# ofsouzap/DistributedMandelbrot

Hardware: AMD Instinct MI355X
Metric: G pixel-iterations/s on 4096^2 tile, max_iter=1000 fp64 (higher is better)
Workload: dtype f64

## Files before the change

### distributedmandelbrot_amd/_lib.py

```python
from __future__ import annotations

import ctypes as C
import importlib.util
import os
import sys

HERE = os.path.dirname(os.path.abspath(__file__))
SO_PATH = os.path.join(HERE, "libmbk_hip.so")

MBK_OK, MBK_ERR_INVALID, MBK_ERR_NO_DEVICE, MBK_ERR_HIP, MBK_ERR_NOMEM, MBK_ERR_NET = range(6)
MBK_WANT_COUNTS = 0x1
MBK_WANT_BYTES = 0x2
MBK_KERNEL_DEFAULT = 0x000
MBK_KERNEL_SIMPLE = 0x100
MBK_KERNEL_ASM = 0x200
MBK_KERNEL_REFILL = 0x300
MBK_KERNEL_GROUP = 0x400
MBK_KERNEL_SCAN = 0x500
KERNELS = {"default": MBK_KERNEL_DEFAULT, "simple": MBK_KERNEL_SIMPLE, "asm": MBK_KERNEL_ASM,
           "refill": MBK_KERNEL_REFILL, "group": MBK_KERNEL_GROUP, "scan": MBK_KERNEL_SCAN}
OPTIONS = {name: i for i, name in enumerate(
    ["order", "waves_per_wg", "group_steps", "exact_steps", "probe_steps", "scan_waves", "scan_xcd_map", "scan_col_period", "heavy_share",
     "rf_livemin", "rf_patience", "rf_batch", "rf_waves", "cycle_detect", "probe_mid", "prepass_overlap", "exact_long", "scan_inline", "wave_limit", "units_min_light", "xcd_balance", "m_late", "h_settled", "classify_wg", "scan_strip", "cycle_window", "spill_first", "spill_lanes", "spill_min_mrd", "spill_min_blocks", "spill_cyc_shift",
     "sure_interior"])}
MBK_PRECISION_F32 = 0x1000
MBK_LAZY_UNIFORM = 0x2000
MBK_DEEP_BLA = 0x8000
MBK_DEEP_XBLA = 0x10000
PRECISIONS = {"f64": 0, "f32": MBK_PRECISION_F32}
MBK_SLOTS = 4
MBK_WORKER_DEPTH = 3
MBK_INFO_SCAN_WG_PER_CU = 100
MBK_INFO_XCD_SHARE = 110
MBK_INFO_SPILL = 130
MBK_CODEC_RAW = 0x00
MBK_CODEC_RLE = 0x01
MBK_CHUNK_DEFINITION = 4096
MBK_CHUNK_BYTES = 4096 * 4096
MBK_ABI_VERSION = 5
MBK_RENDER_BYTES = 0
MBK_RENDER_SMOOTH = 1
MBK_RENDER_DISTANCE = 3
MBK_RENDER_DISTANCE_REL = 4
MBK_RENDER_EQUALIZED = 5
RENDER_SOURCES = {"bytes": MBK_RENDER_BYTES, "smooth": MBK_RENDER_SMOOTH, "distance": MBK_RENDER_DISTANCE,
                  "distance_rel": MBK_RENDER_DISTANCE_REL, "equalized": MBK_RENDER_EQUALIZED}
MBK_HISTOGRAM_MAX_MRD = 1 << 20
# ... 131 lines not shown
    "mbk_view_launch_distance": (C.c_int, [C.c_void_p, C.POINTER(mbk_view), C.c_uint32, C.c_uint32,
                                           C.c_void_p, C.c_void_p, C.c_void_p]),
    "mbk_view_compute_distance": (C.c_int, [C.c_void_p, C.POINTER(mbk_view), C.c_uint32, C.c_uint32,
                                            C.c_void_p, C.c_void_p, C.POINTER(mbk_stats)]),
    "mbk_distance_value_host": (C.c_double, [C.c_double, C.c_double, C.c_int32]),
    "mbk_datachunk_submit": (C.c_int, [C.c_void_p, C.c_int, C.c_uint32, C.c_uint32, C.c_uint32, C.c_uint32,
                                       C.c_void_p, C.c_void_p]),
    "mbk_datachunk_submit_ex": (C.c_int, [C.c_void_p, C.c_int, C.c_uint32, C.c_uint32, C.c_uint32, C.c_uint32,
                                          C.c_void_p, C.c_void_p, C.c_uint32]),
    "mbk_view_submit": (C.c_int, [C.c_void_p, C.c_int, C.POINTER(mbk_view), C.c_uint32, C.c_uint32,
                                  C.c_void_p, C.c_void_p]),
    "mbk_wait": (C.c_int, [C.c_void_p, C.c_int, C.POINTER(mbk_stats)]),
    "mbk_serialize_last": (C.c_int, [C.c_void_p, C.c_void_p, C.c_uint64, C.POINTER(C.c_uint64),
                                     C.POINTER(C.c_uint32)]),
    "mbk_set_option": (C.c_int, [C.c_void_p, C.c_int, C.c_uint32]),
    "mbk_get_option": (C.c_int, [C.c_void_p, C.c_int, C.POINTER(C.c_uint32)]),
    "mbk_quantise_counts": (C.c_int, [C.c_void_p, C.c_void_p, C.c_uint64, C.c_uint32, C.c_void_p]),
    "mbk_units_plan": (C.c_int, [C.c_uint32, C.c_uint32, C.c_uint32, C.c_void_p, C.c_void_p]),
    "mbk_units_lookup": (C.c_int, [C.c_void_p, C.c_uint32, C.c_void_p, C.c_void_p]),
    "mbk_sure_interior_point": (C.c_int, [C.c_double, C.c_double]),
    "mbk_sure_interior_blocks": (C.c_int, [C.POINTER(mbk_view), C.POINTER(C.c_uint64)]),
    "mbk_sure_interior_flag": (C.c_int, [C.POINTER(mbk_view), C.c_uint32, C.c_uint32, C.c_uint32, C.c_uint32,
                                         C.POINTER(C.c_uint32)]),
    "mbk_reduce_counts": (C.c_int, [C.c_void_p, C.c_void_p, C.c_uint64, C.c_uint32, C.c_void_p,
                                    C.POINTER(mbk_stats)]),
    "mbk_worker_run": (C.c_int, [C.c_void_p, C.c_char_p, C.c_uint16, C.c_uint64, C.c_uint32,
                                 C.POINTER(mbk_worker_report)]),
    "mbk_net_set_option": (C.c_int, [C.c_int, C.c_uint32]),
    "mbk_net_get_option": (C.c_int, [C.c_int, C.POINTER(C.c_uint32)]),
    "mbk_feeder_run": (C.c_int, [C.POINTER(mbk_feeder_ops), C.c_char_p, C.c_uint16, C.c_uint64, C.c_uint32,
                                 C.POINTER(mbk_worker_report)]),
    "mbk_deep_orbit_create": (C.c_int, [C.c_char_p, C.c_char_p, C.c_uint32, C.c_uint32, C.POINTER(C.c_void_p)]),
    "mbk_deep_orbit_destroy": (None, [C.c_void_p]),
    "mbk_deep_orbit_info": (C.c_int, [C.c_void_p, C.POINTER(C.c_uint32), C.POINTER(C.c_uint32), C.POINTER(C.c_uint32),
                                      C.POINTER(C.c_uint32)]),
    "mbk_deep_orbit_read": (C.c_int, [C.c_void_p, C.c_void_p, C.c_void_p, C.c_uint64]),
    "mbk_deep_view_launch": (C.c_int, [C.c_void_p, C.c_void_p, C.POINTER(mbk_deep_view), C.c_uint32, C.c_uint32,
                                       C.c_void_p, C.c_void_p, C.c_void_p, C.c_void_p]),
    "mbk_deep_view_compute": (C.c_int, [C.c_void_p, C.c_void_p, C.POINTER(mbk_deep_view), C.c_uint32, C.c_uint32,
                                        C.c_void_p, C.c_void_p, C.c_void_p, C.POINTER(mbk_stats)]),
    "mbk_deep_view_submit": (C.c_int, [C.c_void_p, C.c_int, C.c_void_p, C.POINTER(mbk_deep_view), C.c_uint32, C.c_uint32,
                                       C.c_void_p, C.c_void_p]),
    "mbk_deep_view_launch_distance": (C.c_int, [C.c_void_p, C.c_void_p, C.POINTER(mbk_deep_view), C.c_uint32, C.c_uint32,
                                                C.c_void_p, C.c_void_p, C.c_void_p]),
    "mbk_deep_view_compute_distance": (C.c_int, [C.c_void_p, C.c_void_p, C.POINTER(mbk_deep_view), C.c_uint32, C.c_uint32,
                                                 C.c_void_p, C.c_void_p, C.POINTER(mbk_stats)]),
# ... 299 lines not shown
```

### distributedmandelbrot_amd/csrc/mbk_api.hip

```cpp
#include "../../include/mbk.h"

#include <hip/hip_runtime.h>

#include <cmath>
#include <cstdio>
#include <cstdlib>
#include <algorithm>
#include <cstring>
#include <new>
#include <string>
#include <vector>

#include "mbk_kernels.h"
#include "mbk_refill.h"
#include "mbk_persist.h"
#include "mbk_scan.h"
#include "mbk_units.h"
#include "mbk_spill.h"
#include "mbk_feeder.h"
#include "mbk_deep_orbit.h"
#include "mbk_deep.h"
#include "mbk_deep_bla.h"
#include "mbk_deep_wide.h"
#include "mbk_deep_wide_bla.h"
#include "mbk_histogram.h"
// ... 4 lines not shown
#include "mbk_interior.h"
#include "mbk_deep_distance.h"
#include "mbk_deep_distance_bla.h"
#include "mbk_deep_relief.h"
#include "mbk_deep_nucleus.h"
#include "mbk_deep_wide_nucleus.h"
#include "mbk_deep_wide_distance_bla.h"
#include "mbk_deep_wide_relief.h"
#include "mbk_deep_wide_distance.h"
#include "mbk_julia.h"
#include "mbk_julia_distance.h"
#include "mbk_density.h"
#include "mbk_adaptive.h"
#include "mbk_deep_adaptive.h"
#include "mbk_deep_wide_adaptive.h"

using mbk::Axis;
using mbk::ReduceOut;
using mbk::ReduceSlot;
using mbk::TileArgs;
using mbk::WorkQueues;
using mbk::kSafeImagMin;

static const int kOrderRing = 3;

struct OrderRing {
    uint32_t *d_order[kOrderRing] = {};
    uint32_t *d_capture = nullptr;
    uint32_t *d_ctl = nullptr;
    bool ctl_dirty = true;
    size_t order_cap = 0;
    unsigned order_turn = 0;
    hipStream_t aux = nullptr;
    uint32_t aux_prio = 0;
    int pp_last = -1;
    hipEvent_t ev_cls[kOrderRing] = {};
    hipEvent_t ev_done[kOrderRing] = {};
    bool done_valid[kOrderRing] = {};

    void drop_lists()
    {
        for (int k = 0; k < kOrderRing; ++k) {
            if (d_order[k]) (void)hipFree(d_order[k]);
            d_order[k] = nullptr;
            done_valid[k] = false;
        }
        if (d_capture) (void)hipFree(d_capture);
        d_capture = nullptr;
        order_cap = 0;
    }
    void drop_aux()
    {
        if (aux) (void)hipStreamDestroy(aux);
        aux = nullptr;
        for (int k = 0; k < kOrderRing; ++k) {
            if (ev_cls[k]) (void)hipEventDestroy(ev_cls[k]);
            if (ev_done[k]) (void)hipEventDestroy(ev_done[k]);
            ev_cls[k] = ev_done[k] = nullptr;
            done_valid[k] = false;
        }
    }
    void release()
    {
        if (aux) (void)hipStreamSynchronize(aux);
        drop_lists();
        drop_aux();
        if (d_ctl) (void)hipFree(d_ctl);
        *this = OrderRing();
    }
};

struct SpillBuffers {
    void *d_z = nullptr;
    uint32_t *d_meta = nullptr, *d_cnt = nullptr, *d_chunks = nullptr, *d_src = nullptr;
    unsigned long long *d_total = nullptr;
    size_t cap_slots = 0, cap_blocks = 0;

    void release()
    {
        for (void *q : {d_z, (void *)d_meta, (void *)d_cnt, (void *)d_chunks, (void *)d_src, (void *)d_total})
            if (q) (void)hipFree(q);
        *this = SpillBuffers();
    }
// ... 428 lines not shown
    p.order_mode = ctx->opt[MBK_OPT_ORDER];
    p.probe_steps = ctx->opt[MBK_OPT_PROBE_STEPS];
    a.perm_mul = p.order_mode == 1 ? coprime_multiplier(p.grid.x) : 1u;
    a.order = nullptr;
    p.units = p.order_mode == 3 && p.wpw == 1u && kernel == MBK_KERNEL_GROUP && !safe && a.smooth == nullptr &&
              (a.counts || a.bytes) && !(a.bytes && a.quant_wide) && a.blocks_x % 8u == 0u && a.blocks_x <= 2048u &&
              a.fast_bx_end > 0u && a.fast_by_end > 0u && (f32 || ctx->opt[MBK_OPT_GROUP_STEPS] == 16u) &&
              p.grid.x >= 16384u && (uint32_t)a.mrd > 2u * p.probe_steps && p.by <= 0xffffu;
    p.unit_share = 0.0;
    if (p.units) {
        p.unit_share = window_heavy_share(ctx, a);
        p.units = (1.0 - p.unit_share) * 65536.0 >= (double)ctx->opt[MBK_OPT_UNITS_MIN_LIGHT];
    }
    p.ordered = p.order_mode >= 2 && p.grid.x >= 16384u && (uint32_t)a.mrd > 2u * p.probe_steps && a.blocks_x <= 0xffffu && p.by <= 0xffffu;
    return p;
}

struct OrderList {
    StreamScratch *sc = nullptr;
    unsigned k = 0;
    uint32_t *list = nullptr;
    hipStream_t pre = nullptr;
    bool overlap = false;
    bool whole = false;
    ~OrderList() { if (sc && !whole) sc->ring.ctl_dirty = true; }
};

static const char *capture_list_missing(const OrderRing &ring, uint32_t nblocks, bool units)
{
    if (nblocks > ring.order_cap || !ring.d_capture)
        return "the stream's dispatch lists must grow for this window: make the same call, or a larger one, once outside the capture";
    if (units && (!ring.d_ctl || ring.ctl_dirty))
        return "the units pre-pass' counters must be cleared behind a drain: make the same call once outside the capture";
    return nullptr;
}

static bool capture_list_ready(const mbk_ctx *ctx, hipStream_t stream, uint32_t nblocks, bool units)
{
    for (const StreamScratch &sc : ctx->scratch)
        if (sc.stream == stream) return capture_list_missing(sc.ring, nblocks, units) == nullptr;
    return false;
}

static int acquire_order_list(mbk_ctx *ctx, hipStream_t stream, uint32_t nblocks, bool units, OrderList *out)
{
    StreamScratch *sc = nullptr;
    int rc = get_scratch(ctx, stream, &sc);
    if (rc != MBK_OK) return rc;
    OrderRing &ring = sc->ring;
    if (ctx->capturing) {
        if (const char *why = capture_list_missing(ring, nblocks, units)) return refuse_capture(ctx, why);
        out->k = (unsigned)kOrderRing;
        out->list = ring.d_capture;
        out->pre = stream;
        out->overlap = false;
        out->sc = sc;
        return MBK_OK;
    }
    const uint32_t pp_mode = ctx->opt[MBK_OPT_PREPASS_OVERLAP];
    const bool overlap = pp_mode != 0u;
    const uint32_t want_prio = pp_mode == 2u ? 2u : 1u;
    if (ring.pp_last != (int)pp_mode) {
        if (ring.pp_last >= 0) {
            MBK_HIP(ctx, hipStreamSynchronize(stream));
            if (ring.aux) MBK_HIP(ctx, hipStreamSynchronize(ring.aux));
        }
        for (int k = 0; k < kOrderRing; ++k) ring.done_valid[k] = false;
        ring.pp_last = (int)pp_mode;
    }
    if (overlap && ring.aux && ring.aux_prio != want_prio) {
        MBK_HIP(ctx, hipStreamSynchronize(stream));
        MBK_HIP(ctx, hipStreamSynchronize(ring.aux));
        ring.drop_aux();
    }
    if (overlap && !ring.aux) {
        if (want_prio == 2u) {
            int least = 0, greatest = 0;
            MBK_HIP(ctx, hipDeviceGetStreamPriorityRange(&least, &greatest));
            MBK_HIP(ctx, hipStreamCreateWithPriority(&ring.aux, hipStreamNonBlocking, greatest));
        } else {
            MBK_HIP(ctx, hipStreamCreateWithFlags(&ring.aux, hipStreamNonBlocking));
        }
        ring.aux_prio = want_prio;
        for (int k = 0; k < kOrderRing; ++k) {
            MBK_HIP(ctx, hipEventCreateWithFlags(&ring.ev_cls[k], hipEventDisableTiming));
            MBK_HIP(ctx, hipEventCreateWithFlags(&ring.ev_done[k], hipEventDisableTiming));
        }
    }
    if (nblocks > ring.order_cap) {
        MBK_HIP(ctx, hipStreamSynchronize(stream));
        if (ring.aux) MBK_HIP(ctx, hipStreamSynchronize(ring.aux));
        ring.drop_lists();
        for (int k = 0; k < kOrderRing; ++k)
            MBK_HIP(ctx, hipMalloc((void **)&ring.d_order[k], mbk::units_list_words(nblocks) * sizeof(uint32_t)));
        MBK_HIP(ctx, hipMalloc((void **)&ring.d_capture, mbk::units_list_words(nblocks) * sizeof(uint32_t)));
        ring.order_cap = nblocks;
    }
    const unsigned k = ring.order_turn++ % (unsigned)kOrderRing;
    if (overlap && ring.done_valid[k]) MBK_HIP(ctx, hipStreamWaitEvent(ring.aux, ring.ev_done[k], 0));
    out->k = k;
    out->list = ring.d_order[k];
    out->pre = overlap ? ring.aux : stream;
    out->overlap = overlap;
    out->sc = sc;
    return MBK_OK;
}

static int enqueue_units_prepass(mbk_ctx *ctx, TileArgs &a, const BlockLaunchPlan &p, const OrderList &ol, hipStream_t stream)
{
    StreamScratch *sc = ol.sc;
    OrderRing &ring = sc->ring;
    const uint32_t hs = p.cyc ? ctx->opt[MBK_OPT_H_SETTLED] : 0u;
    const double settle_thr = hs ? std::pow(10.0, -(double)hs) : 0.0;
    if (!ring.d_ctl) {
        MBK_HIP(ctx, hipMalloc((void **)&ring.d_ctl, (size_t)(kOrderRing + 1) * 8u * sizeof(uint32_t)));
        ring.ctl_dirty = true;
    }
    if (ring.ctl_dirty) {
        if (ring.aux) MBK_HIP(ctx, hipStreamSynchronize(ring.aux));
        MBK_HIP(ctx, hipStreamSynchronize(stream));
        MBK_HIP(ctx, hipMemsetAsync(ring.d_ctl, 0, (size_t)(kOrderRing + 1) * 8u * sizeof(uint32_t), ol.pre));
        ring.ctl_dirty = false;
    }
    uint32_t *ctl = ring.d_ctl + 8u * ol.k;
    const uint32_t balance = ctx->opt[MBK_OPT_XCD_BALANCE] == 1u && (p.cyc || ctx->prop.multiProcessorCount != 256 || ctx->capturing)
                                 ? 0u : ctx->opt[MBK_OPT_XCD_BALANCE];
    static const double kUneven[8] = {0.110, 0.140, 0.125, 0.120, 0.130, 0.125, 0.115, 0.135};
    if (balance == 1u && !sc->h_stamps) {
        MBK_HIP(ctx, hipHostMalloc((void **)&sc->h_stamps, (size_t)kStampSlots * mbk::kStampWords * sizeof(unsigned long long),
                                   hipHostMallocDefault));
        std::memset(sc->h_stamps, 0xff, (size_t)kStampSlots * mbk::kStampWords * sizeof(unsigned long long));
    }
    if (balance == 1u) xcd_shares_update(ctx, *sc);
    mbk::XcdShares w;
    double f[8];
    StreamScratch::SharesUsed captured;
    const uint32_t seq = ctx->capturing ? sc->xcd_issued : ++sc->xcd_issued;
    StreamScratch::SharesUsed &used = ctx->capturing ? captured : sc->xcd_ring[seq % kShareRing];
    used.seq = seq;
    used.switches = ctx->stream_switches;
    for (uint32_t x = 0; x < 8u; ++x) {
        f[x] = balance == 1u ? sc->xcd_f[x] : (balance == 2u ? kUneven[x] : 0.125);
        used.f[x] = (float)f[x];
    }
    shares_from_fractions(f, w.cum);
    a.plan = ol.list + ((2u * (size_t)p.grid.x + 5u + 15u) & ~(size_t)15u);
    a.stamps = balance == 1u ? sc->h_stamps + (size_t)(seq % kStampSlots) * mbk::kStampWords : nullptr;
    a.stamp_tag = seq & 0xffffu;
    const uint32_t cwg = ctx->opt[MBK_OPT_CLASSIFY_WG];
    hipLaunchKernelGGL(mbk::classify_units_kernel, dim3((p.grid.x + cwg - 1u) / cwg), dim3(cwg), 0, ol.pre, a, p.grid.x,
                       (int32_t)p.probe_steps, ol.list, ctl, (int32_t)ctx->opt[MBK_OPT_M_LATE], settle_thr, ctl + 3, (uint32_t *)a.plan, w,
                       a.stamps ? 1u : 0u);
    return MBK_OK;
}

static int enqueue_classify_prepass(mbk_ctx *ctx, const TileArgs &a, const BlockLaunchPlan &p, const OrderList &ol, bool *mid_first)
{
    const uint32_t nblocks = p.grid.x;
    uint32_t *cursors = ol.list + nblocks;
    const int rc = clear_words(ctx, cursors, 3u, ol.pre);
    if (rc != MBK_OK) return rc;
    *mid_first = p.order_mode == 3 && ctx->opt[MBK_OPT_PROBE_MID] > p.probe_steps && ctx->opt[MBK_OPT_M_LATE] >= 2u &&
                 ctx->opt[MBK_OPT_M_LATE] <= p.probe_steps;
    hipLaunchKernelGGL(mbk::classify_blocks_kernel, dim3((nblocks + 1023u) / 1024u), dim3(1024), 0, ol.pre, a,
                       nblocks, 8u * p.wpw, (int32_t)p.probe_steps, (int32_t)(*mid_first ? ctx->opt[MBK_OPT_M_LATE] : ctx->opt[MBK_OPT_PROBE_MID]),
                       ol.list, cursors);
    return MBK_OK;
}

static bool spill_wanted(const mbk_ctx *ctx, const TileArgs &a, const BlockLaunchPlan &p, uint32_t kernel, bool safe, bool f32)
{
    const uint32_t spill_first = ctx->opt[MBK_OPT_SPILL_FIRST], spill_lanes = ctx->opt[MBK_OPT_SPILL_LANES];
    return !p.units && a.order != nullptr && p.order_mode >= 2u && kernel == MBK_KERNEL_GROUP && !safe && a.smooth == nullptr && p.wpw == 1u &&
           (a.counts || a.bytes) && spill_first != 0u && (f32 || ctx->opt[MBK_OPT_GROUP_STEPS] == 16u) &&
           (uint32_t)a.mrd >= ctx->opt[MBK_OPT_SPILL_MIN_MRD] && (uint32_t)a.mrd < (1u << 26) &&
           ((uint64_t)p.grid.x >> ctx->opt[MBK_OPT_SPILL_MIN_BLOCKS]) != 0ull &&
           (uint64_t)a.mrd > (uint64_t)ctx->opt[MBK_OPT_EXACT_STEPS] + spill_first + 66u &&
           (uint64_t)p.grid.x * spill_lanes < (1ull << 32) && a.fast_bx_end > 0u && a.fast_by_end > 0u;
}

static int acquire_spill(mbk_ctx *ctx, StreamScratch *sc, hipStream_t stream, TileArgs &a, uint32_t nblocks, SpillBuffers **out)
{
    SpillBuffers &sp = sc->spill;
    const uint32_t spill_lanes = ctx->opt[MBK_OPT_SPILL_LANES];
    const size_t slots = (size_t)nblocks * spill_lanes, nchunks = (nblocks + mbk::kSpillChunk - 1u) / mbk::kSpillChunk;
    *out = nullptr;
    if (slots > sp.cap_slots || nblocks > sp.cap_blocks) {
        MBK_HIP(ctx, hipStreamSynchronize(stream));
        sp.release();
// ... 51 lines not shown
    if (spill) return mbk::tile_asm_kernel<double, true, 16, false, true>;
    if (f32 && safe) return mbk::tile_asm_kernel<float, false, 0>;
    if (f32 && kernel == MBK_KERNEL_ASM) return mbk::tile_asm_kernel<float, true, 0>;
    if (f32 && cyc) return mbk::tile_asm_kernel<float, true, 8, true>;
    if (f32) return mbk::tile_asm_kernel<float, true, 8>;
    if (safe) return mbk::tile_asm_kernel<double, false, 0>;
    if (kernel == MBK_KERNEL_ASM) return mbk::tile_asm_kernel<double, true, 0>;
    if (group_steps == 32 && !cyc) return mbk::tile_asm_kernel<double, true, 32>;
    if (group_steps >= 16 && cyc) return mbk::tile_asm_kernel<double, true, 16, true>;
    if (group_steps >= 16) return mbk::tile_asm_kernel<double, true, 16>;
    if (group_steps == 8 && cyc) return mbk::tile_asm_kernel<double, true, 8, true>;
    if (group_steps == 8) return mbk::tile_asm_kernel<double, true, 8>;
    return mbk::tile_asm_kernel<double, true, 4>;
}

static SpillKernel pick_spill_kernels(bool f32, bool cyc)
{
    if (f32 && cyc) return mbk::tile_spill_kernel<float, true>;
    if (f32) return mbk::tile_spill_kernel<float, false>;
    if (cyc) return mbk::tile_spill_kernel<double, true>;
    return mbk::tile_spill_kernel<double, false>;
}

static void enqueue_units_tile(mbk_ctx *ctx, TileArgs &a, const BlockLaunchPlan &p, bool f32, uint32_t lds, hipStream_t stream, FuseStats *fuse)
{
    const double est = (double)p.grid.x * (p.unit_share + (1.0 - p.unit_share) / 8.0);
    const uint32_t cus = (uint32_t)ctx->prop.multiProcessorCount;
    uint32_t g = (uint32_t)std::min<double>((double)p.grid.x, est * 1.15 + 2048.0);
    g = (std::max(std::max(g, std::min(p.grid.x, cus * 64u)), 16384u) + 7u) & ~7u;
    a.unit_stride = g;
    const bool stats = fuse != nullptr && fuse->slots != nullptr && fuse->counts_unwanted && a.bytes != nullptr;
    if (stats) {
        a.stats = fuse->slots;
        a.counts = nullptr;
        fuse->fused = true;
    }
    hipLaunchKernelGGL(pick_units_kernel(f32, p.cyc, stats, a.counts != nullptr, a.bytes != nullptr), dim3(g), dim3(64), lds, stream, a,
                       quant_table4(a.mrd, a.bytes != nullptr));
}

static int enqueue_spill_second_pass(mbk_ctx *ctx, const TileArgs &a, const SpillBuffers &sp, uint32_t nblocks, bool f32, bool cyc, hipStream_t stream)
{
    const uint32_t nchunks = (nblocks + mbk::kSpillChunk - 1u) / mbk::kSpillChunk;
    hipLaunchKernelGGL(mbk::spill_count_kernel, dim3(nchunks), dim3(mbk::kSpillChunk), 0, stream, sp.d_cnt, nblocks, nchunks, sp.d_chunks);
    hipLaunchKernelGGL(mbk::rle_scan_kernel, dim3(1), dim3(1024), 0, stream, sp.d_chunks, nchunks * mbk::kSpillLevels, sp.d_total);
    hipLaunchKernelGGL(mbk::spill_expand_kernel, dim3(nchunks), dim3(mbk::kSpillChunk), 0, stream, sp.d_cnt, nblocks, nchunks,
                       sp.d_chunks, a.spill_lanes, sp.d_src);
    const uint32_t nwg = (uint32_t)std::min<uint64_t>(((uint64_t)nblocks * a.spill_lanes + 63u) / 64u, 16384u);
    const uint32_t lds2 = 0u;
    hipLaunchKernelGGL(pick_spill_kernels(f32, cyc), dim3(nwg), dim3(64), lds2, stream, a, sp.d_src, sp.d_total, nwg);
    MBK_HIP(ctx, hipGetLastError());
    ++ctx->spill_launches;
    ctx->last_spill_stream = stream;
    return MBK_OK;
}

static int launch_blocks(mbk_ctx *ctx, TileArgs a, uint32_t kernel, bool safe, bool f32, hipStream_t stream, FuseStats *fuse = nullptr,
                         bool list_optional = false)
{
    BlockLaunchPlan p = block_launch_plan(ctx, a, kernel, safe, f32);
    if (p.ordered && list_optional && ctx->capturing && !capture_list_ready(ctx, stream, p.grid.x, p.units)) p.ordered = p.units = false;
    OrderList ol;
    if (p.ordered) {
        int rc = acquire_order_list(ctx, stream, p.grid.x, p.units, &ol);
        if (rc != MBK_OK) return rc;
        OrderRing &ring = ol.sc->ring;
        bool mid_first = false;
        rc = p.units ? enqueue_units_prepass(ctx, a, p, ol, stream) : enqueue_classify_prepass(ctx, a, p, ol, &mid_first);
        if (rc != MBK_OK) return rc;
        if (ol.overlap) {
            MBK_HIP(ctx, hipEventRecord(ring.ev_cls[ol.k], ring.aux));
            MBK_HIP(ctx, hipStreamWaitEvent(stream, ring.ev_cls[ol.k], 0));
        }
        a.order = ol.list;
        a.ngrid = p.grid.x;
        a.order_mid = mid_first ? 2u : (ctx->opt[MBK_OPT_PROBE_MID] <= p.probe_steps ? 1u : 0u);
    }
    SpillBuffers *spill = nullptr;
    if (!ctx->capturing && spill_wanted(ctx, a, p, kernel, safe, f32)) {
        const int rc = acquire_spill(ctx, ol.sc, stream, a, p.grid.x, &spill);
        if (rc != MBK_OK) return rc;
    }
    const uint32_t lds = p.wpw == 1u ? ctx->wave_limit_lds[ctx->opt[MBK_OPT_WAVE_LIMIT] & 7u] : 0u;
    if (p.units && a.order)
        enqueue_units_tile(ctx, a, p, f32, lds, stream, fuse);
    else
        hipLaunchKernelGGL(pick_block_kernel(kernel, safe, f32, p.cyc, ctx->opt[MBK_OPT_GROUP_STEPS], spill != nullptr), p.grid, p.block, lds, stream, a);
    const hipError_t e = hipGetLastError();
    if (e != hipSuccess) return fail(ctx, MBK_ERR_HIP, std::string("tile launch: ") + hipGetErrorString(e));
    if (ol.overlap) {
        MBK_HIP(ctx, hipEventRecord(ol.sc->ring.ev_done[ol.k], stream));
        ol.sc->ring.done_valid[ol.k] = true;
    }
    if (spill) {
        const int rc = enqueue_spill_second_pass(ctx, a, *spill, p.grid.x, f32, p.cyc, stream);
        if (rc != MBK_OK) return rc;
    }
    ol.whole = true;
    return MBK_OK;
}

static bool window_may_touch_ring(const TileArgs &a, double margin = 1e-6)
{
    const double x0 = axis_value_host(a.re, a.col0), x1 = axis_value_host(a.re, a.col0 + a.ncols - 1u);
    const double y0 = axis_value_host(a.im, a.row0), y1 = axis_value_host(a.im, a.row0 + a.nrows - 1u);
    const double xlo = std::fmin(x0, x1), xhi = std::fmax(x0, x1), ylo = std::fmin(y0, y1), yhi = std::fmax(y0, y1);
    const double dx = (xlo <= 0.0 && 0.0 <= xhi) ? 0.0 : std::fmin(std::fabs(xlo), std::fabs(xhi));
    const double dy = (ylo <= 0.0 && 0.0 <= yhi) ? 0.0 : std::fmin(std::fabs(ylo), std::fabs(yhi));
    const double fx = std::fmax(std::fabs(xlo), std::fabs(xhi)), fy = std::fmax(std::fabs(ylo), std::fabs(yhi));
    const double rmin2 = dx * dx + dy * dy, rmax2 = fx * fx + fy * fy;
    return !(rmax2 < 4.0 - margin || rmin2 > 4.0 + margin);
}

static uint32_t sure_interior_word(const TileArgs &a, bool f32, bool cyc, uint32_t option)
{
// ... 760 lines not shown
}

int mbk_create(int device, mbk_ctx **out)
{
    if (!out) return fail(nullptr, MBK_ERR_INVALID, "out is NULL");
    *out = nullptr;
    int n = 0;
    hipError_t e = hipGetDeviceCount(&n);
    if (e != hipSuccess || n <= 0)
        return fail(nullptr, MBK_ERR_NO_DEVICE,
                    std::string("no HIP device visible (") + hipGetErrorString(e) +
                        "); libmbk_hip has no CPU fallback");
    if (device < 0 || device >= n) return fail(nullptr, MBK_ERR_NO_DEVICE, "device index out of range");
    mbk_ctx *ctx = new (std::nothrow) mbk_ctx();
    if (!ctx) return fail(nullptr, MBK_ERR_NOMEM, "out of host memory");
    ctx->device = device;
    static const uint32_t kDefaults[MBK_OPT_COUNT_] = {
         3u,  1u,  16u,  8u,  32u,
         8u,  1u,  4u,  655u,
         48u,  256u,  1u,  8u,  1u,
         65537u,  1u,  0u,  1u,  0u,
         32768u,  0u,  8u,  6u,  1024u,
         1u,  32u,  256u,  16u,  2048u,  19u,  5u,
         1u};
    std::memcpy(ctx->opt, kDefaults, sizeof(kDefaults));
#define MBK_CREATE_HIP(call)                                                        \
    do {                                                                            \
        hipError_t e2_ = (call);                                                    \
        if (e2_ != hipSuccess) {                                                    \
            fail(nullptr, MBK_ERR_HIP, std::string(#call) + ": " + hipGetErrorString(e2_)); \
            mbk_destroy(ctx);                                                       \
            return MBK_ERR_HIP;                                                     \
        }                                                                           \
    } while (0)
    MBK_CREATE_HIP(hipSetDevice(device));
    MBK_CREATE_HIP(hipGetDeviceProperties(&ctx->prop, device));
    if (std::strncmp(ctx->prop.gcnArchName, "gfx950", 6) != 0) {
        fail(nullptr, MBK_ERR_NO_DEVICE,
             std::string("device is ") + ctx->prop.gcnArchName + ", this library is built for gfx950 only");
        mbk_destroy(ctx);
        return MBK_ERR_NO_DEVICE;
    }
    for (Slot &sl : ctx->s) {
        MBK_CREATE_HIP(hipStreamCreateWithFlags(&sl.stream, hipStreamNonBlocking));
        MBK_CREATE_HIP(hipEventCreate(&sl.ev_k0));
        MBK_CREATE_HIP(hipEventCreate(&sl.ev_k1));
        MBK_CREATE_HIP(hipEventCreate(&sl.ev_c0));
// ... 642 lines not shown
        case MBK_OPT_RF_LIVEMIN: ok = value <= 63u; break;
        case MBK_OPT_RF_PATIENCE: ok = value >= 16u && value <= (1u << 20); break;
        case MBK_OPT_RF_BATCH: ok = value >= 1u && value <= 64u; break;
        case MBK_OPT_RF_WAVES: ok = value >= 1u && value <= 8u; break;
        case MBK_OPT_CYCLE_DETECT: ok = value <= 1u; break;
        case MBK_OPT_PROBE_MID: ok = value >= 2u && value <= 65537u; break;
        case MBK_OPT_PREPASS_OVERLAP: ok = value <= 2u; break;
        case MBK_OPT_CLASSIFY_WG: ok = value >= 64u && value <= 1024u && value % 64u == 0u; break;
        case MBK_OPT_SCAN_STRIP: ok = value <= 1u; break;
        case MBK_OPT_CYCLE_WINDOW: ok = value <= 65536u; break;
        case MBK_OPT_EXACT_LONG: ok = value <= 4096u; break;
        case MBK_OPT_SCAN_INLINE: ok = value <= 1u; break;
        case MBK_OPT_WAVE_LIMIT: ok = value <= 7u; break;
        case MBK_OPT_UNITS_MIN_LIGHT: ok = value <= 65536u; break;
        case MBK_OPT_XCD_BALANCE: ok = value <= 2u; break;
        case MBK_OPT_M_LATE: ok = value <= 65536u; break;
        case MBK_OPT_H_SETTLED: ok = value <= 30u; break;
        case MBK_OPT_SPILL_FIRST: ok = value <= 65536u && value % 32u == 0u; break;
        case MBK_OPT_SPILL_LANES: ok = value >= 1u && value <= 32u; break;
        case MBK_OPT_SPILL_MIN_MRD: ok = true; break;
        case MBK_OPT_SPILL_MIN_BLOCKS: ok = value <= 31u; break;
        case MBK_OPT_SPILL_CYC_SHIFT: ok = value <= 31u; break;
        case MBK_OPT_SURE_INTERIOR: ok = value <= 2u; break;
        default: return fail(ctx, MBK_ERR_INVALID, "unknown MBK_OPT_* selector");
    }
    if (!ok) return fail(ctx, MBK_ERR_INVALID, "option value out of range");
    ctx->opt[option] = value;
    return MBK_OK;
}

int mbk_get_option(mbk_ctx *ctx, int option, uint32_t *value)
{
    if (!ctx || !value) return fail(ctx, MBK_ERR_INVALID, "NULL argument");
    if (option >= MBK_INFO_SCAN_WG_PER_CU && option < MBK_INFO_SCAN_WG_PER_CU + 4) {
        const int k = option - MBK_INFO_SCAN_WG_PER_CU;
        *value = (uint32_t)ctx->scan_occ[k >> 1][k & 1];
        return MBK_OK;
    }
    if (option >= MBK_INFO_XCD_SHARE && option < MBK_INFO_XCD_SHARE + 10) {
        const StreamScratch *best = nullptr;
        for (const StreamScratch &sc : ctx->scratch)
            if (!best || sc.xcd_consumed > best->xcd_consumed) best = &sc;
        const int k = option - MBK_INFO_XCD_SHARE;
        *value = !best ? 0u : k < 8 ? (uint32_t)std::lround(best->xcd_f[k] * 1048576.0) : k == 8 ? best->xcd_consumed : best->xcd_issued;
        return MBK_OK;
    }
// ... 28 lines not shown

int mbk_units_plan(uint32_t n_h, uint32_t n_v, uint32_t n_m, const double *fractions, uint32_t *plan)
{
    if (!fractions || !plan) return MBK_ERR_INVALID;
    if ((uint64_t)n_h + n_v + n_m > 0x7fffffffull) return MBK_ERR_INVALID;
    uint32_t cum[8];
    shares_from_fractions(fractions, cum);
    mbk::units_plan(n_h, n_v, n_m, cum, 0u, plan, 0u, 0u);
    return MBK_OK;
}

int mbk_units_lookup(const uint32_t *plan, uint32_t id, uint32_t *list, uint32_t *index)
{
    if (!plan || !list || !index) return MBK_ERR_INVALID;
    const uint32_t x = id & 7u;
    bool is_h = false;
    uint32_t i = 0;
    *list = 0u;
    *index = 0u;
    if (id >= plan[2] || !mbk::units_lookup(id, plan[3], plan[4], plan[8u + x], plan[16u + x], plan[24u + x], plan[32u + x], is_h, i))
        return MBK_OK;
    *list = is_h ? 1u : (i < plan[1] ? 2u : 3u);
    *index = is_h ? i : (i < plan[1] ? i : i - plan[1]);
    return MBK_OK;
}

int mbk_sure_interior_point(double cr, double ci) { return mbk::sure_interior_point(cr, ci) ? 1 : 0; }

int mbk_sure_interior_blocks(const mbk_view *view, uint64_t *certified)
{
    if (!view || !certified) return fail(nullptr, MBK_ERR_INVALID, "NULL argument");
    bool safe = false;
    const int rc = validate_view(nullptr, view, &safe);
    if (rc != MBK_OK) return rc;
    TileArgs a = view_window_args(view);
    set_window_facts(a, false);
    uint64_t n = 0;
    for (uint32_t by = 0; by < a.fast_by_end; ++by)
        for (uint32_t bx = 0; bx < a.fast_bx_end; ++bx) {
            bool all = true;
            for (uint32_t ly = 0; ly < 8u && all; ++ly) {
                const double ci = (double)(a.row0 + by * 8u + ly) * a.im.step + a.im.start;
                for (uint32_t lx = 0; lx < 8u && all; ++lx)
                    all = mbk::sure_interior_point((double)(a.col0 + bx * 8u + lx) * a.re.step + a.re.start, ci);
            }
            n += all ? 1u : 0u;
// ... 3566 lines not shown
```

### include/mbk.h

```cpp
#ifndef MBK_H
#define MBK_H

#include <stdint.h>

#ifdef __cplusplus
extern "C" {
#endif

#define MBK_ABI_VERSION 5

#define MBK_CHUNK_DEFINITION 4096u
#define MBK_CHUNK_BYTES (4096u * 4096u)

enum mbk_status {
    MBK_OK = 0,
    MBK_ERR_INVALID = 1,
    MBK_ERR_NO_DEVICE = 2,
    MBK_ERR_HIP = 3,
    MBK_ERR_NOMEM = 4,
    MBK_ERR_NET = 5
};

#define MBK_WANT_COUNTS 0x1u
#define MBK_WANT_BYTES 0x2u
// ... 479 lines not shown
    MBK_OPT_RF_LIVEMIN,
    MBK_OPT_RF_PATIENCE,
    MBK_OPT_RF_BATCH,
    MBK_OPT_RF_WAVES,
    MBK_OPT_CYCLE_DETECT,
    MBK_OPT_PROBE_MID,
    MBK_OPT_PREPASS_OVERLAP,
    MBK_OPT_EXACT_LONG,
    MBK_OPT_SCAN_INLINE,
    MBK_OPT_WAVE_LIMIT,
    MBK_OPT_UNITS_MIN_LIGHT,
    MBK_OPT_XCD_BALANCE,
    MBK_OPT_M_LATE,
    MBK_OPT_H_SETTLED,
    MBK_OPT_CLASSIFY_WG,
    MBK_OPT_SCAN_STRIP,
    MBK_OPT_CYCLE_WINDOW,
    MBK_OPT_SPILL_FIRST,
    MBK_OPT_SPILL_LANES,
    MBK_OPT_SPILL_MIN_MRD,
    MBK_OPT_SPILL_MIN_BLOCKS,
    MBK_OPT_SPILL_CYC_SHIFT,
    MBK_OPT_SURE_INTERIOR,
    MBK_OPT_COUNT_
};
#define MBK_INFO_SCAN_WG_PER_CU 100
#define MBK_INFO_XCD_SHARE 110
#define MBK_INFO_SPILL 130
int mbk_set_option(mbk_ctx *ctx, int option, uint32_t value);
int mbk_get_option(mbk_ctx *ctx, int option, uint32_t *value);

int mbk_units_plan(uint32_t n_h, uint32_t n_v, uint32_t n_m, const double *fractions, uint32_t *plan);
int mbk_units_lookup(const uint32_t *plan, uint32_t id, uint32_t *list, uint32_t *index);

int mbk_sure_interior_point(double cr, double ci);
int mbk_sure_interior_blocks(const mbk_view *view, uint64_t *certified);
int mbk_sure_interior_flag(const mbk_view *view, uint32_t mrd, uint32_t flags, uint32_t cycle_detect, uint32_t option,
                           uint32_t *flag);

int mbk_quantise_counts(mbk_ctx *ctx, const int32_t *h_counts, uint64_t n, uint32_t mrd, uint8_t *h_bytes);

int mbk_reduce_counts(mbk_ctx *ctx, const int32_t *d_counts, uint64_t n, uint32_t mrd,
                      void *hip_stream, mbk_stats *stats);

typedef struct mbk_worker_report {
    uint64_t leased;
    uint64_t accepted;
    uint64_t rejected;
    uint64_t resets;
    uint64_t uniform_tiles;
    uint64_t pixel_iterations;
    double kernel_ms_sum;
    double seconds;
    uint64_t net_retries;
} mbk_worker_report;
int mbk_worker_run(mbk_ctx *ctx, const char *addr, uint16_t port, uint64_t max_tiles, uint32_t senders,
                   mbk_worker_report *report);

enum mbk_net_option {
    MBK_NET_MAX_CONNECTIONS = 0,
    MBK_NET_CONNECT_TIMEOUT_MS = 1,
// ... 27 lines not shown
```

Before: 5413.

## Deepen order-list ring and record completion events at kernel dispatch with periodic guards

Grows the prepass order-list ring from 3 to 8 buffers and adds an order_guard option (default 1) under which only every fourth tile launch records a done event. Classify and tile kernels signal their events through hipExtLaunchKernelGGL stop events instead of separate hipEventRecord calls. The aim is to cut per-tile event record and wait overhead between the auxiliary prepass stream and the main stream, so the prepass can run further ahead. In exchange it uses more order-list memory, adds a full-stream fallback fence when no matching record exists, and makes reuse safety depend on the period-to-ring arithmetic.

```diff
diff --git a/distributedmandelbrot_amd/_lib.py b/distributedmandelbrot_amd/_lib.py
--- a/distributedmandelbrot_amd/_lib.py
+++ b/distributedmandelbrot_amd/_lib.py
@@ -22,7 +22,7 @@
 OPTIONS = {name: i for i, name in enumerate(
     ["order", "waves_per_wg", "group_steps", "exact_steps", "probe_steps", "scan_waves", "scan_xcd_map", "scan_col_period", "heavy_share",
      "rf_livemin", "rf_patience", "rf_batch", "rf_waves", "cycle_detect", "probe_mid", "prepass_overlap", "exact_long", "scan_inline", "wave_limit", "units_min_light", "xcd_balance", "m_late", "h_settled", "classify_wg", "scan_strip", "cycle_window", "spill_first", "spill_lanes", "spill_min_mrd", "spill_min_blocks", "spill_cyc_shift",
-     "sure_interior"])}
+     "sure_interior", "order_guard"])}
 MBK_PRECISION_F32 = 0x1000
 MBK_LAZY_UNIFORM = 0x2000
 MBK_DEEP_BLA = 0x8000
@@ -200,6 +200,7 @@
     "mbk_sure_interior_blocks": (C.c_int, [C.POINTER(mbk_view), C.POINTER(C.c_uint64)]),
     "mbk_sure_interior_flag": (C.c_int, [C.POINTER(mbk_view), C.c_uint32, C.c_uint32, C.c_uint32, C.c_uint32,
                                          C.POINTER(C.c_uint32)]),
+    "mbk_order_guard_host": (C.c_int, [C.c_uint64, C.c_uint32, C.c_uint32, C.POINTER(C.c_int64), C.POINTER(C.c_uint32)]),
     "mbk_reduce_counts": (C.c_int, [C.c_void_p, C.c_void_p, C.c_uint64, C.c_uint32, C.c_void_p,
                                     C.POINTER(mbk_stats)]),
     "mbk_worker_run": (C.c_int, [C.c_void_p, C.c_char_p, C.c_uint16, C.c_uint64, C.c_uint32,
diff --git a/distributedmandelbrot_amd/csrc/mbk_api.hip b/distributedmandelbrot_amd/csrc/mbk_api.hip
--- a/distributedmandelbrot_amd/csrc/mbk_api.hip
+++ b/distributedmandelbrot_amd/csrc/mbk_api.hip
@@ -1,6 +1,7 @@
 #include "../../include/mbk.h"
 
 #include <hip/hip_runtime.h>
+#include <hip/hip_ext.h>
 
 #include <cmath>
 #include <cstdio>
@@ -51,7 +52,21 @@
 using mbk::WorkQueues;
 using mbk::kSafeImagMin;
 
-static const int kOrderRing = 3;
+static const int kOrderRing = 8;
+
+static inline bool order_guard_legal(uint32_t R, uint32_t P) { return R >= 2u && P >= 1u && P <= R / 2u; }
+static inline void order_guard_event(uint64_t turn, uint32_t R, uint32_t P, int64_t *wait_turn, bool *records)
+{
+    *records = (turn + 1u) % P == 0u;
+    *wait_turn = turn < R ? -1 : (int64_t)(((turn - R) / P + 1u) * P - 1u);
+}
+
+static inline void order_guard_shape(uint32_t guard, uint32_t *R, uint32_t *P, bool *on_dispatch)
+{
+    *R = guard == 1u ? (uint32_t)kOrderRing : guard == 2u ? 2u : 3u;
+    *P = guard == 1u ? 4u : 1u;
+    *on_dispatch = guard != 0u;
+}
 
 struct OrderRing {
     uint32_t *d_order[kOrderRing] = {};
@@ -59,24 +74,35 @@
     uint32_t *d_ctl = nullptr;
     bool ctl_dirty = true;
     size_t order_cap = 0;
-    unsigned order_turn = 0;
+    uint32_t lists = 0;
+    uint64_t order_turn = 0;
+    uint64_t guard_base = 0;
     hipStream_t aux = nullptr;
     uint32_t aux_prio = 0;
     int pp_last = -1;
+    int guard_last = -1;
     hipEvent_t ev_cls[kOrderRing] = {};
     hipEvent_t ev_done[kOrderRing] = {};
+    hipEvent_t ev_full = nullptr;
     bool done_valid[kOrderRing] = {};
-
+    uint64_t done_turn[kOrderRing] = {};
+
+    void forget_records()
+    {
+        for (int k = 0; k < kOrderRing; ++k) done_valid[k] = false;
+        guard_base = order_turn;
+    }
     void drop_lists()
     {
         for (int k = 0; k < kOrderRing; ++k) {
             if (d_order[k]) (void)hipFree(d_order[k]);
             d_order[k] = nullptr;
-            done_valid[k] = false;
         }
+        forget_records();
         if (d_capture) (void)hipFree(d_capture);
         d_capture = nullptr;
         order_cap = 0;
+        lists = 0;
     }
     void drop_aux()
     {
@@ -86,8 +112,10 @@
             if (ev_cls[k]) (void)hipEventDestroy(ev_cls[k]);
             if (ev_done[k]) (void)hipEventDestroy(ev_done[k]);
             ev_cls[k] = ev_done[k] = nullptr;
-            done_valid[k] = false;
         }
+        if (ev_full) (void)hipEventDestroy(ev_full);
+        ev_full = nullptr;
+        forget_records();
     }
     void release()
     {
@@ -562,6 +590,9 @@
     uint32_t *list = nullptr;
     hipStream_t pre = nullptr;
     bool overlap = false;
+    bool on_dispatch = false;
+    bool records = false;
+    uint64_t turn = 0;
     bool whole = false;
     ~OrderList() { if (sc && !whole) sc->ring.ctl_dirty = true; }
 };
@@ -600,13 +631,18 @@
     const uint32_t pp_mode = ctx->opt[MBK_OPT_PREPASS_OVERLAP];
     const bool overlap = pp_mode != 0u;
     const uint32_t want_prio = pp_mode == 2u ? 2u : 1u;
-    if (ring.pp_last != (int)pp_mode) {
+    const uint32_t guard = ctx->opt[MBK_OPT_ORDER_GUARD];
+    uint32_t R = 0, P = 0;
+    bool on_dispatch = false;
+    order_guard_shape(guard, &R, &P, &on_dispatch);
+    if (ring.pp_last != (int)pp_mode || ring.guard_last != (int)guard) {
         if (ring.pp_last >= 0) {
             MBK_HIP(ctx, hipStreamSynchronize(stream));
             if (ring.aux) MBK_HIP(ctx, hipStreamSynchronize(ring.aux));
         }
-        for (int k = 0; k < kOrderRing; ++k) ring.done_valid[k] = false;
+        ring.forget_records();
         ring.pp_last = (int)pp_mode;
+        ring.guard_last = (int)guard;
     }
     if (overlap && ring.aux && ring.aux_prio != want_prio) {
         MBK_HIP(ctx, hipStreamSynchronize(stream));
@@ -626,25 +662,57 @@
             MBK_HIP(ctx, hipEventCreateWithFlags(&ring.ev_cls[k], hipEventDisableTiming));
             MBK_HIP(ctx, hipEventCreateWithFlags(&ring.ev_done[k], hipEventDisableTiming));
         }
-    }
-    if (nblocks > ring.order_cap) {
+        MBK_HIP(ctx, hipEventCreateWithFlags(&ring.ev_full, hipEventDisableTiming));
+    }
+    if (nblocks > ring.order_cap || R > ring.lists) {
         MBK_HIP(ctx, hipStreamSynchronize(stream));
         if (ring.aux) MBK_HIP(ctx, hipStreamSynchronize(ring.aux));
+        const size_t cap = std::max<size_t>(nblocks, ring.order_cap);
+        const uint32_t lists = std::max(R, ring.lists);
         ring.drop_lists();
-        for (int k = 0; k < kOrderRing; ++k)
-            MBK_HIP(ctx, hipMalloc((void **)&ring.d_order[k], mbk::units_list_words(nblocks) * sizeof(uint32_t)));
-        MBK_HIP(ctx, hipMalloc((void **)&ring.d_capture, mbk::units_list_words(nblocks) * sizeof(uint32_t)));
-        ring.order_cap = nblocks;
-    }
-    const unsigned k = ring.order_turn++ % (unsigned)kOrderRing;
-    if (overlap && ring.done_valid[k]) MBK_HIP(ctx, hipStreamWaitEvent(ring.aux, ring.ev_done[k], 0));
+        for (uint32_t k = 0; k < lists; ++k)
+            MBK_HIP(ctx, hipMalloc((void **)&ring.d_order[k], mbk::units_list_words(cap) * sizeof(uint32_t)));
+        MBK_HIP(ctx, hipMalloc((void **)&ring.d_capture, mbk::units_list_words(cap) * sizeof(uint32_t)));
+        ring.order_cap = cap;
+        ring.lists = lists;
+    }
+    const uint64_t turn = ring.order_turn++;
+    const unsigned k = (unsigned)(turn % R);
+    int64_t wait_turn = -1;
+    bool records = false;
+    order_guard_event(turn, R, P, &wait_turn, &records);
+    if (overlap && wait_turn >= (int64_t)ring.guard_base) {
+        const unsigned kw = (unsigned)((uint64_t)wait_turn % R);
+        if (ring.done_valid[kw] && ring.done_turn[kw] == (uint64_t)wait_turn) {
+            MBK_HIP(ctx, hipStreamWaitEvent(ring.aux, ring.ev_done[kw], 0));
+            ring.guard_base = (uint64_t)wait_turn + 1u;
+        } else {
+            MBK_HIP(ctx, hipEventRecord(ring.ev_full, stream));
+            MBK_HIP(ctx, hipStreamWaitEvent(ring.aux, ring.ev_full, 0));
+            ring.guard_base = turn;
+        }
+    }
     out->k = k;
     out->list = ring.d_order[k];
     out->pre = overlap ? ring.aux : stream;
     out->overlap = overlap;
+    out->on_dispatch = overlap && on_dispatch;
+    out->records = overlap && records;
+    out->turn = turn;
     out->sc = sc;
     return MBK_OK;
 }
+
+template <typename... Formal, typename... Args>
+static void launch_with_stop(void (*kernel)(Formal...), dim3 grid, dim3 block, uint32_t lds, hipStream_t stream, hipEvent_t stop, Args... args)
+{
+    if (stop)
+        hipExtLaunchKernelGGL(kernel, grid, block, lds, stream, nullptr, stop, 0u, args...);
+    else
+        hipLaunchKernelGGL(kernel, grid, block, lds, stream, args...);
+}
+
+static hipEvent_t prepass_stop_event(const OrderList &ol) { return ol.overlap && ol.on_dispatch ? ol.sc->ring.ev_cls[ol.k] : nullptr; }
 
 static int enqueue_units_prepass(mbk_ctx *ctx, TileArgs &a, const BlockLaunchPlan &p, const OrderList &ol, hipStream_t stream)
 {
@@ -688,9 +756,9 @@
     a.stamps = balance == 1u ? sc->h_stamps + (size_t)(seq % kStampSlots) * mbk::kStampWords : nullptr;
     a.stamp_tag = seq & 0xffffu;
     const uint32_t cwg = ctx->opt[MBK_OPT_CLASSIFY_WG];
-    hipLaunchKernelGGL(mbk::classify_units_kernel, dim3((p.grid.x + cwg - 1u) / cwg), dim3(cwg), 0, ol.pre, a, p.grid.x,
-                       (int32_t)p.probe_steps, ol.list, ctl, (int32_t)ctx->opt[MBK_OPT_M_LATE], settle_thr, ctl + 3, (uint32_t *)a.plan, w,
-                       a.stamps ? 1u : 0u);
+    launch_with_stop(mbk::classify_units_kernel, dim3((p.grid.x + cwg - 1u) / cwg), dim3(cwg), 0, ol.pre, prepass_stop_event(ol), a, p.grid.x,
+                     (int32_t)p.probe_steps, ol.list, ctl, (int32_t)ctx->opt[MBK_OPT_M_LATE], settle_thr, ctl + 3, (uint32_t *)a.plan, w,
+                     a.stamps ? 1u : 0u);
     return MBK_OK;
 }
 
@@ -702,9 +770,9 @@
     if (rc != MBK_OK) return rc;
     *mid_first = p.order_mode == 3 && ctx->opt[MBK_OPT_PROBE_MID] > p.probe_steps && ctx->opt[MBK_OPT_M_LATE] >= 2u &&
                  ctx->opt[MBK_OPT_M_LATE] <= p.probe_steps;
-    hipLaunchKernelGGL(mbk::classify_blocks_kernel, dim3((nblocks + 1023u) / 1024u), dim3(1024), 0, ol.pre, a,
-                       nblocks, 8u * p.wpw, (int32_t)p.probe_steps, (int32_t)(*mid_first ? ctx->opt[MBK_OPT_M_LATE] : ctx->opt[MBK_OPT_PROBE_MID]),
-                       ol.list, cursors);
+    launch_with_stop(mbk::classify_blocks_kernel, dim3((nblocks + 1023u) / 1024u), dim3(1024), 0, ol.pre, prepass_stop_event(ol), a,
+                     nblocks, 8u * p.wpw, (int32_t)p.probe_steps, (int32_t)(*mid_first ? ctx->opt[MBK_OPT_M_LATE] : ctx->opt[MBK_OPT_PROBE_MID]),
+                     ol.list, cursors);
     return MBK_OK;
 }
 
@@ -802,7 +870,8 @@
     return mbk::tile_spill_kernel<double, false>;
 }
 
-static void enqueue_units_tile(mbk_ctx *ctx, TileArgs &a, const BlockLaunchPlan &p, bool f32, uint32_t lds, hipStream_t stream, FuseStats *fuse)
+static void enqueue_units_tile(mbk_ctx *ctx, TileArgs &a, const BlockLaunchPlan &p, bool f32, uint32_t lds, hipStream_t stream, FuseStats *fuse,
+                               hipEvent_t stop)
 {
     const double est = (double)p.grid.x * (p.unit_share + (1.0 - p.unit_share) / 8.0);
     const uint32_t cus = (uint32_t)ctx->prop.multiProcessorCount;
@@ -815,8 +884,8 @@
         a.counts = nullptr;
         fuse->fused = true;
     }
-    hipLaunchKernelGGL(pick_units_kernel(f32, p.cyc, stats, a.counts != nullptr, a.bytes != nullptr), dim3(g), dim3(64), lds, stream, a,
-                       quant_table4(a.mrd, a.bytes != nullptr));
+    launch_with_stop(pick_units_kernel(f32, p.cyc, stats, a.counts != nullptr, a.bytes != nullptr), dim3(g), dim3(64), lds, stream, stop, a,
+                     quant_table4(a.mrd, a.bytes != nullptr));
 }
 
 static int enqueue_spill_second_pass(mbk_ctx *ctx, const TileArgs &a, const SpillBuffers &sp, uint32_t nblocks, bool f32, bool cyc, hipStream_t stream)
@@ -849,7 +918,7 @@
         rc = p.units ? enqueue_units_prepass(ctx, a, p, ol, stream) : enqueue_classify_prepass(ctx, a, p, ol, &mid_first);
         if (rc != MBK_OK) return rc;
         if (ol.overlap) {
-            MBK_HIP(ctx, hipEventRecord(ring.ev_cls[ol.k], ring.aux));
+            if (!ol.on_dispatch) MBK_HIP(ctx, hipEventRecord(ring.ev_cls[ol.k], ring.aux));
             MBK_HIP(ctx, hipStreamWaitEvent(stream, ring.ev_cls[ol.k], 0));
         }
         a.order = ol.list;
@@ -862,15 +931,18 @@
         if (rc != MBK_OK) return rc;
     }
     const uint32_t lds = p.wpw == 1u ? ctx->wave_limit_lds[ctx->opt[MBK_OPT_WAVE_LIMIT] & 7u] : 0u;
+    const hipEvent_t done_stop = ol.records && ol.on_dispatch ? ol.sc->ring.ev_done[ol.k] : nullptr;
     if (p.units && a.order)
-        enqueue_units_tile(ctx, a, p, f32, lds, stream, fuse);
+        enqueue_units_tile(ctx, a, p, f32, lds, stream, fuse, done_stop);
     else
-        hipLaunchKernelGGL(pick_block_kernel(kernel, safe, f32, p.cyc, ctx->opt[MBK_OPT_GROUP_STEPS], spill != nullptr), p.grid, p.block, lds, stream, a);
+        launch_with_stop(pick_block_kernel(kernel, safe, f32, p.cyc, ctx->opt[MBK_OPT_GROUP_STEPS], spill != nullptr), p.grid, p.block, lds, stream,
+                         done_stop, a);
     const hipError_t e = hipGetLastError();
     if (e != hipSuccess) return fail(ctx, MBK_ERR_HIP, std::string("tile launch: ") + hipGetErrorString(e));
-    if (ol.overlap) {
-        MBK_HIP(ctx, hipEventRecord(ol.sc->ring.ev_done[ol.k], stream));
+    if (ol.records) {
+        if (!ol.on_dispatch) MBK_HIP(ctx, hipEventRecord(ol.sc->ring.ev_done[ol.k], stream));
         ol.sc->ring.done_valid[ol.k] = true;
+        ol.sc->ring.done_turn[ol.k] = ol.turn;
     }
     if (spill) {
         const int rc = enqueue_spill_second_pass(ctx, a, *spill, p.grid.x, f32, p.cyc, stream);
@@ -1677,7 +1749,7 @@
          65537u,  1u,  0u,  1u,  0u,
          32768u,  0u,  8u,  6u,  1024u,
          1u,  32u,  256u,  16u,  2048u,  19u,  5u,
-         1u};
+         1u,  1u};
     std::memcpy(ctx->opt, kDefaults, sizeof(kDefaults));
 #define MBK_CREATE_HIP(call)                                                        \
     do {                                                                            \
@@ -2366,6 +2438,7 @@
         case MBK_OPT_SPILL_MIN_BLOCKS: ok = value <= 31u; break;
         case MBK_OPT_SPILL_CYC_SHIFT: ok = value <= 31u; break;
         case MBK_OPT_SURE_INTERIOR: ok = value <= 2u; break;
+        case MBK_OPT_ORDER_GUARD: ok = value <= 2u; break;
         default: return fail(ctx, MBK_ERR_INVALID, "unknown MBK_OPT_* selector");
     }
     if (!ok) return fail(ctx, MBK_ERR_INVALID, "option value out of range");
@@ -2440,6 +2513,16 @@
         return MBK_OK;
     *list = is_h ? 1u : (i < plan[1] ? 2u : 3u);
     *index = is_h ? i : (i < plan[1] ? i : i - plan[1]);
+    return MBK_OK;
+}
+
+int mbk_order_guard_host(uint64_t turn, uint32_t ring, uint32_t period, int64_t *wait_turn, uint32_t *records)
+{
+    if (!wait_turn || !records) return fail(nullptr, MBK_ERR_INVALID, "NULL argument");
+    if (!order_guard_legal(ring, period)) return fail(nullptr, MBK_ERR_INVALID, "order guard: the period must lie in 1 .. ring / 2");
+    bool rec = false;
+    order_guard_event(turn, ring, period, wait_turn, &rec);
+    *records = rec ? 1u : 0u;
     return MBK_OK;
 }
 
diff --git a/include/mbk.h b/include/mbk.h
--- a/include/mbk.h
+++ b/include/mbk.h
@@ -525,6 +525,7 @@
     MBK_OPT_SPILL_MIN_BLOCKS,
     MBK_OPT_SPILL_CYC_SHIFT,
     MBK_OPT_SURE_INTERIOR,
+    MBK_OPT_ORDER_GUARD,
     MBK_OPT_COUNT_
 };
 #define MBK_INFO_SCAN_WG_PER_CU 100
@@ -540,6 +541,8 @@
 int mbk_sure_interior_blocks(const mbk_view *view, uint64_t *certified);
 int mbk_sure_interior_flag(const mbk_view *view, uint32_t mrd, uint32_t flags, uint32_t cycle_detect, uint32_t option,
                            uint32_t *flag);
+
+int mbk_order_guard_host(uint64_t turn, uint32_t ring, uint32_t period, int64_t *wait_turn, uint32_t *records);
 
 int mbk_quantise_counts(mbk_ctx *ctx, const int32_t *h_counts, uint64_t n, uint32_t mrd, uint8_t *h_bytes);
 
```

New measurement: 5447, median of 6. About the same (+0.6%).
